# Zain-Jiang/Dict-TTS

Measured on AMD Instinct MI355X. Metric: mel-frames/sec, end-to-end text->mel->wav (audio-samples/sec = 256x; RTF reported alongside), higher is better.
Workload: dtype f16 (vocoder ResBlocks fp16 MFMA, serial convolutions bf16 hi/lo split; acoustic model fp32-grade: fp32 MFMA / bf16 three-piece operands x 6 products)

## Files before the change

### dict_tts_amd/csrc/rblock.hip

```cpp
#include "rblock.h"
#include "rb_common.h"
#include "rb_tiles.h"

#include <algorithm>
#include <type_traits>
#include <cstdlib>

namespace dtts {

#ifdef RB_STAMP
__device__ unsigned long long rb_stamps[2][12][16];
extern "C" __attribute__((visibility("default"))) int dtts_debug_rb_stamps(unsigned long long* host, int reset) {
    hipError_t e = hipMemcpyFromSymbol(host, HIP_SYMBOL(rb_stamps), sizeof(rb_stamps));
    if (e == hipSuccess && reset) {
        static unsigned long long z[2][12][16];
        e = hipMemcpyToSymbol(HIP_SYMBOL(rb_stamps), z, sizeof z);
    }
    return (int)e;
}
#define RB_T(k) do { const unsigned long long _n = __builtin_amdgcn_s_memrealtime(); tq[k] += _n - t_last; t_last = _n; } while (0)
#else
#define RB_T(k)
#endif

template <int C, int MT, int NT, int WT, int WC, int EL, int PS, bool GUARD, class SH = MfmaShape<32>>
__global__ __launch_bounds__(64 * WT * WC, (64 * WT * WC <= 256) ? 2 : 1) void rblock_kernel(const RBlockParams p) {
    static_assert(WC * NT * 32 == C, "channel tiling must cover C");
    typedef typename SH::acc_t acc_t;
    extern __shared__ __attribute__((aligned(16))) char smem[];
    constexpr int THREADS = 64 * WT * WC;
    constexpr int W = 32 * MT * WT;
    constexpr int PITCH = C * 2 + 16;
    constexpr int NKG = C / SH::CI;
    constexpr int EP = C * 4 + 16;
    constexpr int F4 = C / 4, SROWS = WT * 32;
    constexpr size_t ACT_BYTES = (size_t)(W + 2 * RB_GUARD) * PITCH;
    char* act = smem;
    char* stage = smem + ACT_BYTES;

    int tid = threadIdx.x, lane = tid & 63, wave = tid >> 6;
    int wt = wave % WT, wc = wave / WT;
    const int H = rblock_halo(p);
    const int TT = W - 2 * H;
    constexpr int PK = 7, PH = (PK - 1) / 2;
    const int TTo = p.wav ? TT - 2 * PH : TT;

    const RbTiles tiles{(int*)(smem + p.pre_off), p.B};
    auto zero_guard_bands = [&](int t) {
        for (int idx = t; idx < 2 * RB_GUARD * (PITCH / 16); idx += THREADS) {
            const int r = idx / (PITCH / 16), c = idx % (PITCH / 16);
            const int row = r < RB_GUARD ? r : W + r;
            *(uint4*)(act + row * PITCH + c * 16) = make_uint4(0, 0, 0, 0);
        }
    };
    zero_guard_bands(tid);
    int total = 0, j = blockIdx.x;
    if constexpr (PS) {
        tiles.build(p.lens, p.T, TTo, tid, THREADS);
        total = tiles.total();
        if (j >= total) return;
    }
    const int G = gridDim.x;

    typedef __attribute__((ext_vector_type(4))) unsigned int u32x4;
    constexpr int RPP = THREADS / F4;
    constexpr int PER = SROWS / RPP;
    static_assert(THREADS % F4 == 0 && SROWS % RPP == 0, "row-coalesced staging");
    int c4 = tid % F4, r0 = tid / F4;
    auto tile_row = [&](int m, int u) { const int sr = r0 + RPP * u; return ((sr >> 5) * MT + m) * 32 + (sr & 31); };

    auto load_x = [&](acc_t (&d)[NT], int m, int bb, int base, int ln) {
        const auto rs = __builtin_amdgcn_make_buffer_rsrc((void*)(p.x + (long long)bb * p.T * C), 0, ln * C * 4, 0x00020000);
        const int o0 = ((base + wt * MT * 32 + SH::row(lane, 0)) * C + wc * NT * 32 + SH::chan(lane, 0)) * 4;
#pragma unroll
        for (int n = 0; n < NT; ++n)
#pragma unroll
            for (int q = 0; q < 4; ++q) {
                const u32x4 v = __builtin_amdgcn_raw_buffer_load_b128(rs, o0 + (m * 32 * C + n * 32 + SH::row(0, q) * C + SH::chan(0, q)) * 4, 0, RB_X_AUX);
                SH::set_quad(d[n], q, __builtin_bit_cast(f32x4, v));
            }
    };

    int b = 0, len, t0;
    if constexpr (PS) {
        tiles.locate(j, b);
        len = tiles.len_of(b);
        t0 = tiles.first_row(j, b, TTo) - (p.wav ? PH : 0);
    } else {
        b = blockIdx.y;
        len = __builtin_amdgcn_readfirstlane(p.lens ? p.lens[b] : p.T);
        t0 = blockIdx.x * TTo - (p.wav ? PH : 0);
        if (t0 + (p.wav ? PH : 0) >= len) return;
    }
    acc_t xr[MT][NT];
    if constexpr (PS) {
#pragma unroll
        for (int m = 0; m < MT; ++m) load_x(xr[m], m, b, t0 - H, len);
    } else {
        const auto rs_x = __builtin_amdgcn_make_buffer_rsrc((void*)(p.x + (long long)b * p.T * C), 0, len * C * 4, 0x00020000);
        const int g0 = ((t0 - H + r0) * C + c4 * 4) * 4;
        u32x4 ld[MT][PER] = {};
#pragma unroll
        for (int m = 0; m < MT; ++m)
#pragma unroll
            for (int u = 0; u < PER; ++u) ld[m][u] = __builtin_amdgcn_raw_buffer_load_b128(rs_x, g0 + (tile_row(m, u) - r0) * (C * 4), 0, RB_X_AUX);
#pragma unroll
        for (int m = 0; m < MT; ++m) {
            if (m) __syncthreads();
#pragma unroll
            for (int u = 0; u < PER; ++u) *(u32x4*)(stage + (r0 + RPP * u) * EP + c4 * 16) = ld[m][u];
            __syncthreads();
#pragma unroll
            for (int n = 0; n < NT; ++n)
#pragma unroll
                for (int q = 0; q < 4; ++q)
                    SH::set_quad(xr[m][n], q, *(const f32x4*)(stage + (wt * 32 + SH::row(lane, q)) * EP + ((wc * NT + n) * 32 + SH::chan(lane, q)) * 4));
        }
    }

    const int kg_stride = (C / 32) * SH::WF * 64;
    int r = 0;

#ifdef RB_STAMP
    unsigned long long tq[16] = {0, 0, 0, 0, 0, 0, 0, 0, 0, 0, 0, 0, 0, 0, 0, 0};
    unsigned long long t_last = __builtin_amdgcn_s_memrealtime();
#endif
#pragma unroll 1
    for (;;) {
    if constexpr (PS) {
        tid = threadIdx.x;
        asm volatile("" : "+v"(tid));
        lane = tid & 63, wave = __builtin_amdgcn_readfirstlane(tid >> 6);
        wt = wave % WT, wc = wave / WT;
        c4 = tid % F4, r0 = tid / F4;
    }
    const int xlane = (RB_GUARD + wt * MT * 32 + SH::row(lane, 0)) * PITCH + SH::chan(lane, 0) * 4;
    const size_t wlane = (size_t)(wc * NT) * SH::WF * 64 + lane;
    if constexpr (PS) r = __builtin_amdgcn_readfirstlane(r);
    else r = 0;
    const RBlockParams::Set& R = p.rb[PS ? r : 0];
    const int Kr = R.K;
    constexpr bool REAL_STEPS = (C == 32);
    static_assert(!REAL_STEPS || SH::FRAG == 32, "rb2_contract is written for 32x32x16");
    static_assert(REAL_STEPS || NKG >= 4 || (NKG == 2 && SH::FRAG == 16), "whole groups of four k-steps, or rb_contract's half group");
    const int S = (REAL_STEPS ? Kr : R.Kp) * NKG;
    const bool last_rb = !PS || r + 1 == p.nrb;
    const int mode = (!PS || p.nrb == 1 || r == 0) ? p.mode : (last_rb ? p.last_mode : 1);
    const bool wav_now = p.wav && last_rb;
    t0 = __builtin_amdgcn_readfirstlane(t0);
    const int base_t = t0 - H;
    const long long brow = (long long)b * p.T;
    unsigned claim = 0;
    if (PS && p.tile_ctr && tid == 0 && last_rb) claim = atomicAdd(p.tile_ctr, 1u);
    int jn = j + G;
    bool has_next = PS && jn < total;
    int bn = b, lenn = len, t0n = 0;
    auto plan_next = [&]() {
        if (!last_rb) {
            has_next = true;
            jn = j;
            bn = b;
            lenn = len;
            t0n = t0;
            return;
        }
        has_next = PS && jn < total;
        bn = b;
        if (has_next) {
            tiles.locate(jn, bn);
            lenn = tiles.len_of(bn);
            t0n = tiles.first_row(jn, bn, TTo) - (p.wav ? PH : 0);
        }
    };
    if (!(PS && p.tile_ctr) || !last_rb) plan_next();
    const auto rs_s = p.s_private ? __builtin_amdgcn_make_buffer_rsrc((void*)p.S, 0, p.s_private, 0x00020000)
                                  : __builtin_amdgcn_make_buffer_rsrc((void*)(p.S + brow * C), 0, len * C * 4, 0x00020000);

    constexpr int NBQ = 4 / SH::QB;
    auto load_bias = [&](f32x4 (&bb)[NT][NBQ], const float* bias) {
#pragma unroll
        for (int n = 0; n < NT; ++n)
#pragma unroll
            for (int q = 0; q < NBQ; ++q) bb[n][q] = *(const f32x4*)(bias + (wc * NT + n) * 32 + SH::chan(lane, q * SH::QB));
    };
    const bool all_inb = base_t >= 0 && base_t + W <= len;
    int n_ovf = 0;
    auto write_act_impl = [&](char* dst, const acc_t (&v)[MT][NT], auto masked_tag) {
        constexpr bool MASKED = decltype(masked_tag)::value;
        int ln = lane;
        if constexpr (SH::FRAG == 16) asm volatile("" : "+v"(ln));
#pragma unroll
        for (int m = 0; m < MT; ++m) {
            int row[SH::QB];
            bool inb[SH::QB], counted[SH::QB];
#pragma unroll
            for (int rh = 0; rh < SH::QB; ++rh) {
                row[rh] = (wt * MT + m) * 32 + SH::row(ln, rh);
                const int t = base_t + row[rh];
                inb[rh] = !MASKED || (t >= 0 && t < len);
                counted[rh] = inb[rh] && row[rh] >= H && row[rh] < H + TT;
            }
#pragma unroll
            for (int n = 0; n < NT; ++n)
#pragma unroll
                for (int q = 0; q < 4; ++q) {
                    constexpr int QBM = SH::QB - 1;
                    const int co = (wc * NT + n) * 32 + SH::chan(ln, q);
                    const f32x4 v4 = SH::quad(v[m][n], q);
                    uint2 pk = act4<EL>(v4, 0.1f);
                    if constexpr (GUARD) n_ovf += counted[q & QBM] ? ovf4(v4, 0.1f) : 0;
                    if constexpr (MASKED) {
                        if (!inb[q & QBM]) pk = make_uint2(0, 0);
                    }
                    *(uint2*)(dst + (RB_GUARD + row[q & QBM]) * PITCH + co * 2) = pk;
                }
        }
    };
    auto write_act = [&](char* dst, const acc_t (&v)[MT][NT]) {
        if (all_inb) write_act_impl(dst, v, std::false_type{});
        else write_act_impl(dst, v, std::true_type{});
    };

    uint4 ring[SH::RD][NT * SH::WF];
    f32x4 bb[NT][NBQ];
    RB_T(10);
    rb_preload(ring, R.w1[0] + wlane, kg_stride);
    load_bias(bb, R.b1[0]);
    write_act(act, xr);
    RB_T(0);
    __syncthreads();
    RB_T(1);

    acc_t acc[MT][NT];
#pragma unroll 1
    for (int it = 0; it < 3; ++it) {
        acc_t cinit[NT];
#pragma unroll
        for (int n = 0; n < NT; ++n)
#pragma unroll
            for (int q = 0; q < 4; ++q) SH::set_quad(cinit[n], q, bb[n][q / SH::QB]);
        load_bias(bb, R.b2[it]);
        const int d = R.dil[it];
        if constexpr (REAL_STEPS) {
            if (S) rb2_contract<EL, MT, NT, NKG, PITCH, 4, true>(acc, ring, act, xlane - ((Kr - 1) / 2) * d * PITCH, R.w1[it] + wlane, S, d * PITCH, cinit);
            else rb_contract<EL, MT, NT, NKG, PITCH, true, 1>(acc, ring, act, 0, R.w1[it] + wlane, 0, 0, &cinit);
        } else
            rb_contract<EL, MT, NT, NKG, PITCH, true, 1, SH>(acc, ring, act, xlane - ((Kr - 1) / 2) * d * PITCH, R.w1[it] + wlane, S, d * PITCH, &cinit);
        rb_preload(ring, R.w2[it] + wlane, kg_stride);
        RB_T(2);
        __syncthreads();
        RB_T(3);
        write_act(act, acc);
        RB_T(4);
        __syncthreads();
        RB_T(5);
#pragma unroll
        for (int m = 0; m < MT; ++m)
#pragma unroll
            for (int n = 0; n < NT; ++n)
#pragma unroll
                for (int q = 0; q < 4; ++q) SH::add_quad(xr[m][n], q, bb[n][q / SH::QB]);
        if (it < 2) load_bias(bb, R.b1[it + 1]);
        if constexpr (REAL_STEPS) {
            if (S) rb2_contract<EL, MT, NT, NKG, PITCH, 4, false>(xr, ring, act, xlane - ((Kr - 1) / 2) * PITCH, R.w2[it] + wlane, S, PITCH, cinit);
        } else
            rb_contract<EL, MT, NT, NKG, PITCH, false, 1, SH>(xr, ring, act, xlane - ((Kr - 1) / 2) * PITCH, R.w2[it] + wlane, S, PITCH);
        if (it < 2) rb_preload(ring, R.w1[it + 1] + wlane, kg_stride);
        if (PS && p.tile_ctr && last_rb && it == 2 && tid == 0) tiles.publish_claim(G, claim);
        RB_T(6);
        __syncthreads();
        RB_T(7);
        if (it < 2) {
            write_act(act, xr);
            RB_T(0);
            __syncthreads();
            RB_T(1);
        }
    }

    if (PS && p.tile_ctr && last_rb) {
        jn = tiles.claimed();
        plan_next();
    }
    {
    const auto rs_a = __builtin_amdgcn_make_buffer_rsrc((void*)(p.Sa ? p.Sa + brow * C : (unsigned short*)(p.S + brow * C)), 0,
                                                        len * C * 2, 0x00020000);
    constexpr int CW = NT * 32, F4W = CW / 4, RPI = 64 / F4W, NRD = 32 / RPI;
    const int er = lane / F4W, ec = lane % F4W;
    const int goffw = (p.s_private ? (j * TT - H) * C : base_t * C) * 4 + (wc * CW + ec * 4) * 4;
    static_assert(F4W == 8 && RPI == 8 && NRD == 4, "the conflict-free row order below is for 8 lanes per row, 8 rows per access");
    const int erow_slab_base = C == 32 ? er : (er >> 2) + ((er & 1) ? 16 : 0) + ((er & 2) ? 8 : 0);
    auto srow = [&](int u) { return (C == 32 ? 8 : 2) * u + erow_slab_base; };
    auto erow = [&](int m, int u) { return (wt * MT + m) * 32 + srow(u); };
    auto eoff = [&](int m, int u) {
        const int row = erow(m, u);
        return (row >= H && row < H + TT) ? goffw + row * (C * 4) : (int)0x80000000;
    };
    u32x4 sold[MT][NRD];
#pragma unroll
    for (int m = 0; m < MT; ++m)
#pragma unroll
        for (int u = 0; u < NRD; ++u) {
            sold[m][u] = u32x4{0u, 0u, 0u, 0u};
            if (mode >= 1) sold[m][u] = p.nrb > 1 ? __builtin_amdgcn_raw_buffer_load_b128(rs_s, eoff(m, u), 0, 0)
                                                  : __builtin_amdgcn_raw_buffer_load_b128(rs_s, eoff(m, u), 0, VP_LD_AUX);
        }
    RB_T(12);
    constexpr int OP = C * 4;
    char* otile = smem;
    char* estage = wav_now ? smem + ((size_t)TT * OP > ACT_BYTES ? (size_t)TT * OP : ACT_BYTES) : stage;
    char* stg = estage + (wt * 32) * EP + (wc * CW) * 4;
#pragma unroll
    for (int m = 0; m < MT; ++m) {
#pragma unroll
        for (int n = 0; n < NT; ++n)
#pragma unroll
            for (int q = 0; q < 4; ++q) *(f32x4*)(stg + SH::row(lane, q) * EP + (n * 32 + SH::chan(lane, q)) * 4) = SH::quad(xr[m][n], q);
        if (has_next) load_x(xr[m], m, bn, t0n - H, lenn);
        __builtin_amdgcn_fence(__ATOMIC_RELEASE, "wavefront");
        __builtin_amdgcn_wave_barrier();
        __builtin_amdgcn_fence(__ATOMIC_ACQUIRE, "wavefront");
        RB_T(13);
#pragma unroll
        for (int u = 0; u < NRD; ++u) {
            const int off = eoff(m, u);
            f32x4 o = *(const f32x4*)(stg + srow(u) * EP + ec * 16);
            o += __builtin_bit_cast(f32x4, sold[m][u]);
            if (wav_now) {
                const int row = erow(m, u);
                if (row >= H && row < H + TT) {
                    const int t = base_t + row;
#pragma unroll
                    for (int e = 0; e < 4; ++e) o[e] = (t >= 0 && t < len) ? lrelu(o[e] / p.div, p.slope) : 0.f;
                    *(f32x4*)(otile + (size_t)(row - H) * OP + (wc * CW + ec * 4) * 4) = o;
                }
                continue;
            }
            rb_stage_row(o, rs_s, rs_a, off, mode, p.div, p.slope, p.drop_S != 0, p.Sa != nullptr, p.nrb > 1 && !last_rb);
        }
        __builtin_amdgcn_fence(__ATOMIC_RELEASE, "wavefront");
        __builtin_amdgcn_wave_barrier();
        __builtin_amdgcn_fence(__ATOMIC_ACQUIRE, "wavefront");
        RB_T(14);
    }
    if constexpr (C == 32) if (wav_now) {
        __syncthreads();
        rb_conv_post_tanh<C, THREADS, 3>(otile, p.post_w, p.post_b, p.wav + brow, t0, TTo, len, p.bad, tid);
    }
    }
    RB_T(8);
#ifdef RB_STAMP
    tq[11] += 1;
#endif
    if constexpr (GUARD) {
        if (n_ovf) atomicAdd(p.ovf, (unsigned long long)n_ovf);
    }
    if (!has_next) break;
    r = last_rb ? 0 : r + 1;
    if (wav_now) {
        __syncthreads();
        zero_guard_bands(threadIdx.x);
    }
    j = jn;
    b = bn;
    len = lenn;
    t0 = t0n;
    }
#ifdef RB_STAMP
    {
        const int w = threadIdx.x >> 6;
        if ((threadIdx.x & 63) == 0 && (w == 0 || w == WT * WC - 1)) {
            const int slot = (C == 32 ? 0 : C == 64 ? 1 : C == 128 ? 2 : 3) * 3 + (p.K == 3 ? 0 : p.K == 7 ? 1 : 2);
            for (int k = 0; k < 16; ++k) atomicAdd(&rb_stamps[w == 0 ? 0 : 1][slot][k], tq[k]);
        }
    }
#endif
}

template <int C, int MT, int WT>
static size_t rb_lds_bytes(int TT, bool wav) {
    constexpr int W = 32 * MT * WT, PITCH = C * 2 + 16, EP = C * 4 + 16;
    constexpr size_t ACT = (size_t)(W + 2 * RB_GUARD) * PITCH;
    if (wav)
        return std::max((size_t)TT * C * 4, ACT) + (size_t)WT * 32 * EP;
    return ACT + (size_t)WT * 32 * EP;
}

template <int C, int MT, int NT, int WT, int WC, int EL, int PS, bool GUARD = false>
static hipError_t rb_launch_cfg(const RBlockParams& p, hipStream_t stream) {
    typedef MfmaShape<rblock_mfma_shape(C)> SH;
    constexpr int W = 32 * MT * WT;
    for (int j = 0; j < p.nrb; ++j)
        if (!(p.rb[j].K & 1) || p.rb[j].Kp != rblock_padded_taps(C, p.rb[j].K)) return hipErrorInvalidValue;
    const int H = rblock_halo(p), TT = W - 2 * H;
    if (TT < 32) return hipErrorInvalidValue;
    if ((long long)p.T * C * 4 >= (1LL << 31)) return hipErrorInvalidValue;
    if (p.wav && (C != 32 || (p.nrb == 1 && p.mode != 2) || !p.post_w || !p.post_b)) return hipErrorInvalidValue;
    size_t lds = rb_lds_bytes<C, MT, WT>(TT, p.wav != nullptr);
    const int TTo = p.wav ? TT - 6 : TT;
    RBlockParams q = p;
    q.pre_off = (int)lds;
    if (PS) lds += rb_table_bytes(p.B);
    if (lds > 160 * 1024) return hipErrorOutOfMemory;
    constexpr bool HAS_GUARD = !(C == 64 && MT == 5);
    if constexpr (EL == EL_F16 && !GUARD && HAS_GUARD) {
        if (p.ovf) return rb_launch_cfg<C, MT, NT, WT, WC, EL, PS, true>(p, stream);
    }
    if (EL == EL_F16 && !HAS_GUARD && p.ovf) return hipErrorInvalidValue;
    constexpr auto kern = rblock_kernel<C, MT, NT, WT, WC, EL, PS, GUARD, SH>;
    if (const hipError_t e = rb_allow_full_lds<kern>(); e != hipSuccess) return e;
    constexpr int THREADS = 64 * WT * WC;
    if (!PS) {
        hipLaunchKernelGGL(kern, dim3((p.T + TTo - 1) / TTo, p.B), dim3(THREADS), lds, stream, q);
        return hipGetLastError();
    }
    const int cus = rb_device_cus();
    if (cus <= 0) return hipErrorInvalidDevice;
    const int grid = rb_resident_grid(cus, lds, THREADS, THREADS <= 256 ? 2 : 1, (long long)p.B * ((p.T + TTo - 1) / TTo));
    if (grid <= 0) return hipSuccess;
    hipLaunchKernelGGL(kern, dim3(grid), dim3(THREADS), lds, stream, q);
    return hipGetLastError();
}

bool rblock_supported(int C, int K) {
    if (!(K & 1) || K < 3 || K > 11) return false;
    return C == 32 || C == 64 || ((C == 128 || C == 256) && K == 3);
}

int rblock_stage_tile_rows(int C, int halo) {
    return (C == 32 ? 1024 : 512) - 2 * halo;
}

bool rblock_stage_launch_fits(int C, int halo, int B, bool wav) {
    const int TT = rblock_stage_tile_rows(C, halo);
    if (C != 32 && C != 64) return false;
    const size_t lds = (C == 32 ? rb_lds_bytes<32, 4, 8>(TT, wav) : rb_lds_bytes<64, 4, 4>(TT, wav)) + rb_table_bytes(B);
    return TT >= 32 && lds <= 160 * 1024;
}

long long rblock_private_rows(int C, int halo, int B, int T) {
    if (C != 32) return 0;
    const int TT = rblock_stage_tile_rows(C, halo), TTo = TT - 6;
    if (TTo < 32) return 0;
    return (long long)B * ((T + TTo - 1) / TTo) * TT;
}

int rblock_padded_taps(int C, int K) {
    const int sh = rblock_mfma_shape(C);
    const int nkg = C / (sh == 16 ? 32 : 16);
    if (sh == 16 && nkg == 2) return K;
    int kp = K;
    while ((kp * nkg) % 4) ++kp;
    return kp;
}

template <int EL>
static hipError_t rb_launch_el(const RBlockParams& p, int C, hipStream_t stream) {
    const int cus = rb_device_cus();
    if (cus <= 0) return hipErrorInvalidDevice;
    auto few = [&](int W) {
        const int tt = W - 2 * rblock_halo(p) - (p.wav ? 6 : 0);
        return tt >= 32 && 2 * (long long)p.B * ((p.T + tt - 1) / tt) <= cus;
    };
    if (p.nrb < 1 || p.nrb > 3) return hipErrorInvalidValue;
    if (p.nrb > 1) {
        if (C == 32) return rb_launch_cfg<32, 4, 1, 8, 1, EL, 1>(p, stream);
        if (C == 64) return rb_launch_cfg<64, 4, 1, 4, 2, EL, 1>(p, stream);
        return hipErrorInvalidValue;
    }
    if (C == 32 && p.K >= 7 && !few(1024)) RB_TRY((rb_launch_cfg<32, 4, 1, 8, 1, EL, 1>(p, stream)));
    if (C == 64 && few(512)) return rb_launch_cfg<64, 4, 1, 2, 2, EL, 1>(p, stream);
    if (C == 128 && few(256)) return rb_launch_cfg<128, 4, 1, 1, 4, EL, 1>(p, stream);
    if (C == 256 && few(128)) return rb_launch_cfg<256, 2, 1, 1, 8, EL, 1>(p, stream);
    if (C == 32) return rb_launch_cfg<32, 4, 1, 4, 1, EL, 0>(p, stream);
    if (C == 64 && p.K >= 7 && !p.small_tile && !(EL == EL_F16 && p.ovf)) RB_TRY((rb_launch_cfg<64, 5, 1, 4, 2, EL, 1>(p, stream)));
    if (C == 64) RB_TRY((rb_launch_cfg<64, 4, 1, 4, 2, EL, 1>(p, stream)));
    if (C == 64) return rb_launch_cfg<64, 4, 1, 2, 2, EL, 1>(p, stream);
    if (C == 128) RB_TRY((rb_launch_cfg<128, 4, 1, 2, 4, EL, 1>(p, stream)));
    if (C == 128) return rb_launch_cfg<128, 4, 1, 1, 4, EL, 1>(p, stream);
    if (C == 256) RB_TRY((rb_launch_cfg<256, 4, 1, 1, 8, EL, 1>(p, stream)));
    if (C == 256) return rb_launch_cfg<256, 2, 1, 1, 8, EL, 1>(p, stream);
    return hipErrorInvalidValue;
}

hipError_t rblock_launch(const RBlockParams& p, int C, int frag, hipStream_t stream) {
    if (C != 32 && C != 64 && C != 128 && C != 256) return hipErrorInvalidValue;
    if (frag != rblock_mfma_shape(C)) return hipErrorInvalidValue;
    return p.el == EL_F16 ? rb_launch_el<EL_F16>(p, C, stream) : rb_launch_el<EL_BF16>(p, C, stream);
}

}
```

### dict_tts_amd/csrc/vocoder.hip

```cpp
#include "ctx.h"

using namespace dtts;

namespace {

bool vocoder_fp16_analysis(dtts_ctx* h, Need& need) {
    const dtts_config& c = h->cfg;
    const std::string v = "vocoder.";
    const int nk = c.n_resblock_kernels;
    std::vector<double> pt_wc[2], pt_m2[2];
    for (int pass = 0; pass < 2; ++pass) {
        const double M = pass, bs = pass == 0 ? 1.0 : 0.0;
        auto conv = [&](const std::string& base, const std::vector<double>& uin, const std::vector<double>& min, std::vector<double>& uout,
                        std::vector<double>& mout) -> bool {
            const HostTensor* w = folded_weight(h, need, base);
            const std::vector<float> b = bias_of(need, base);
            if (!w || b.empty() || w->shape.size() != 3) return false;
            const int co_n = (int)w->shape[0], ci_n = (int)w->shape[1], k_n = (int)w->shape[2];
            if ((int)uin.size() < ci_n) return false;
            uout.assign(co_n, 0.0);
            mout.assign(co_n, 0.0);
            for (int co = 0; co < co_n; ++co) {
                double su = bs * std::fabs((double)b[co]), sm = bs * (double)b[co] * b[co];
                for (int ci = 0; ci < ci_n; ++ci) {
// ... 3 lines not shown
                        a1 += std::fabs((double)pw[k]);
                        a2 += (double)pw[k] * pw[k];
                    }
                    su += a1 * uin[ci];
                    sm += a2 * min[ci];
                }
                uout[co] = su;
                mout[co] = sm;
            }
            return true;
        };
        std::vector<double> u(c.audio_num_mel_bins, M), m(c.audio_num_mel_bins, M * M), u2, m2;
        if (!conv(v + "conv_pre", u, m, u2, m2)) return false;
        u.swap(u2);
        m.swap(m2);
        for (int i = 0; i < c.n_upsamples; ++i) {
            const int r = c.upsample_rates[i], k_n = c.upsample_kernel_sizes[i], pad = (k_n - r) / 2;
            const HostTensor* w = folded_weight(h, need, v + "ups." + std::to_string(i));
            const std::vector<float> b = bias_of(need, v + "ups." + std::to_string(i));
            if (!w || b.empty() || w->shape.size() != 3 || (int)w->shape[2] != k_n) return false;
            const int ci_n = (int)w->shape[0], co_n = (int)w->shape[1];
            std::vector<double> ux(co_n, 0.0), mx(co_n, 0.0);
            for (int co = 0; co < co_n; ++co)
                for (int ph = 0; ph < r; ++ph) {
                    double su = bs * std::fabs((double)b[co]), sm = bs * (double)b[co] * b[co];
                    for (int ci = 0; ci < ci_n; ++ci) {
                        const float* pw = &w->f[((size_t)ci * co_n + co) * k_n];
                        double a1 = 0, a2 = 0;
                        for (int k = (ph + pad) % r; k < k_n; k += r) {
                            a1 += std::fabs((double)pw[k]);
                            a2 += (double)pw[k] * pw[k];
                        }
                        su += a1 * u[ci];
                        sm += a2 * 0.505 * m[ci];
                    }
                    ux[co] = std::max(ux[co], su);
                    mx[co] = std::max(mx[co], sm);
                }
            std::vector<double> us(co_n, 0.0), ms(co_n, 0.0);
            for (int j = 0; j < nk; ++j) {
                std::vector<double> x = ux, xm = mx, xt, xtm, y, ym, xa(co_n), xam(co_n);
                const std::string rb = v + "resblocks." + std::to_string(i * nk + j);
                for (int mth = 0; mth < (h->resblock2 ? 2 : 3); ++mth) {
                    for (int q = 0; q < co_n; ++q) {
                        pt_wc[pass].push_back(x[q]);
                        pt_m2[pass].push_back(xm[q]);
                        xa[q] = x[q];
                        xam[q] = 0.505 * xm[q];
                    }
                    if (h->resblock2) {
                        if (!conv(rb + ".convs." + std::to_string(mth), xa, xam, y, ym)) return false;
                    } else {
                        if (!conv(rb + ".convs1." + std::to_string(mth), xa, xam, xt, xtm)) return false;
                        for (int q = 0; q < co_n; ++q) {
                            pt_wc[pass].push_back(xt[q]);
                            pt_m2[pass].push_back(xtm[q]);
                            xtm[q] *= 0.505;
                        }
                        if (!conv(rb + ".convs2." + std::to_string(mth), xt, xtm, y, ym)) return false;
                    }
                    for (int q = 0; q < co_n; ++q) {
                        x[q] += y[q];
                        xm[q] += ym[q];
                    }
                }
                for (int q = 0; q < co_n; ++q) {
                    us[q] += x[q] / nk;
                    ms[q] += xm[q] / nk;
                }
            }
            u.swap(us);
            m.swap(ms);
        }
    }
    if (pt_wc[0].size() != pt_wc[1].size()) return false;
    double a_wc = 0, b_wc = 0, a_m2 = 0, b_m2 = 0;
    for (size_t q = 0; q < pt_wc[0].size(); ++q) {
        a_wc = std::max(a_wc, pt_wc[0][q]);
        b_wc = std::max(b_wc, pt_wc[1][q]);
        a_m2 = std::max(a_m2, pt_m2[0][q]);
        b_m2 = std::max(b_m2, pt_m2[1][q]);
    }
    h->wc_const = a_wc;
    h->wc_lin = b_wc;
    h->est_const = std::sqrt(a_m2);
    h->est_lin = std::sqrt(b_m2);
    return true;
}

bool pack_rb_fused(dtts_ctx* h, Need& need, PackedConv& L, int eng, const std::string& base, int ch, int k, int dil, int frag) {
    const HostTensor* w = folded_weight(h, need, base);
    std::vector<float> bias = bias_of(need, base);
    if (!w || bias.empty()) return false;
    const float* pw = w->f.data();
    const int slack = ch >= 64 ? 1 : 2;
    const bool ok = pack_conv(h, L, eng, ch, ch, frag == RBN_FRAG ? rbn_padded_taps(ch, k) : rblock_padded_taps(ch, k) + slack,
                              [=](int co, int ci, int tap) { return tap < k ? pw[((size_t)co * ch + ci) * k + tap] : 0.f; }, bias, dil, 1, 0, 0, -1, frag);
    L.K = k;
    return ok;
}

bool vpair_pack_fits(const PackedConv& L, int ch, int k) {
    return L.C_in == ch && L.C_out == ch && L.C_in_pad == ch && L.C_out_pad == ch && L.K == k && L.frag == vpair_mfma_shape(ch);
}
bool vpair_runs(const dtts_config& c, bool resblock2, int eng_rb, int ch, int k, int d0, int d1, int d2) {
    const bool fuse = c.vocoder_precision == DTTS_VOC_F16 || !c.vocoder_unfused;
    return fuse && !resblock2 && eng_rb != ENG_BF16X3 && !rblock_supported(ch, k) && vpair_supported(ch, k, d0) && vpair_supported(ch, k, d1) &&
           vpair_supported(ch, k, d2);
}

}

namespace dtts {

int build_vocoder(dtts_ctx* h) {
    Need need{h, ""};
    const dtts_config& c = h->cfg;
    if (c.vocoder_precision != DTTS_VOC_BF16 && c.vocoder_precision != DTTS_VOC_BF16X3 && c.vocoder_precision != DTTS_VOC_F16)
        return fail(h, DTTS_E_INVAL, "vocoder_precision %d is not one of DTTS_VOC_BF16 / _BF16X3 / _F16", c.vocoder_precision);
    if (c.vocoder_precision == DTTS_VOC_F16 && c.audio_num_mel_bins % 4)
        return fail(h, DTTS_E_INVAL, "DTTS_VOC_F16 needs audio_num_mel_bins %% 4 == 0 (got %d); use DTTS_VOC_BF16X3", c.audio_num_mel_bins);
    if (!h->ovf_dev) {
        if (!(h->ovf_dev = (unsigned long long*)dev_alloc(h, sizeof(unsigned long long))) || hipMemset(h->ovf_dev, 0, sizeof(unsigned long long)) != hipSuccess)
            return fail(h, DTTS_E_NOMEM, "range-guard counter");
    }
    if (!h->bad_dev) {
        if (!(h->bad_dev = (unsigned*)dev_alloc(h, sizeof(unsigned))) || hipMemset(h->bad_dev, 0, sizeof(unsigned)) != hipSuccess)
            return fail(h, DTTS_E_NOMEM, "overflow-detector counter");
        void* hp = nullptr;
        if (hipHostMalloc(&hp, 64, hipHostMallocDefault) != hipSuccess) return fail(h, DTTS_E_NOMEM, "overflow-detector host word");
        h->bad_host = (volatile unsigned*)hp;
        *h->bad_host = 0;
    }
    const int eng = c.vocoder_precision == DTTS_VOC_BF16 ? ENG_BF16 : ENG_BF16X3;
    const int eng_rb = c.vocoder_precision == DTTS_VOC_F16 ? ENG_F16 : eng;
    const std::string v = "vocoder.";
    bool ok = pack_plain(h, need, h->conv_pre, eng, v + "conv_pre", 1, 1, 3);
    h->ups.resize(c.n_upsamples);
    h->hop = 1;
    for (int i = 0; ok && i < c.n_upsamples; ++i) {
        const int u = c.upsample_rates[i], k = c.upsample_kernel_sizes[i];
        const bool h2 = c.vocoder_precision == DTTS_VOC_F16 && i == 1 && DTTS_TUNE(h, 8192) && (u * (c.upsample_initial_channel >> (i + 1))) % 256 == 0 &&
                        (c.upsample_initial_channel >> i) % 128 == 0;
        ok = ok && pack_transposed(h, need, h->ups[i], h2 ? ENG_F16 : eng, v + "ups." + std::to_string(i), u, (k - u) / 2);
        h->hop *= u;
    }
    const int nk = c.n_resblock_kernels;
    h->rb1.assign((size_t)c.n_upsamples * nk, {});
    h->rb2.assign((size_t)c.n_upsamples * nk, {});
    const bool rb2x = h->resblock2;
    for (int i = 0; ok && i < c.n_upsamples * nk; ++i) {
        const int j = i % nk, k = c.resblock_kernel_sizes[j], n = rb2x ? 2 : 3;
        const int ch = c.upsample_initial_channel >> (i / nk + 1);
        const std::string r = v + "resblocks." + std::to_string(i);
        const int* dl = c.resblock_dilation_sizes[j];
        const bool vp = vpair_runs(c, rb2x, eng_rb, ch, k, dl[0], dl[1], dl[2]);
        const int frag = vp ? vpair_mfma_shape(ch) : 32;
        h->rb1[i].resize(n);
        if (!rb2x) h->rb2[i].resize(3);
        for (int mth = 0; ok && mth < n; ++mth) {
            const int d = c.resblock_dilation_sizes[j][mth];
            ok = ok && pack_plain(h, need, h->rb1[i][mth], eng_rb, r + (rb2x ? ".convs." : ".convs1.") + std::to_string(mth), d, 1, (k * d - d) / 2, true, 0, frag);
            if (!rb2x) ok = ok && pack_plain(h, need, h->rb2[i][mth], eng_rb, r + ".convs2." + std::to_string(mth), 1, 1, (k - 1) / 2, true, 0, frag);
            if (ok && vp && !vpair_pack_fits(h->rb1[i][mth], ch, k))
                return fail(h, DTTS_E_INVAL, "%s%d: weight shape [%d, %d, %d] is not the configured [%d, %d, %d]", (r + ".convs1.").c_str(), mth, h->rb1[i][mth].C_out,
                            h->rb1[i][mth].C_in, h->rb1[i][mth].K, ch, ch, k);
            if (ok && vp && !vpair_pack_fits(h->rb2[i][mth], ch, k))
                return fail(h, DTTS_E_INVAL, "%s%d: weight shape [%d, %d, %d] is not the configured [%d, %d, %d]", (r + ".convs2.").c_str(), mth, h->rb2[i][mth].C_out,
                            h->rb2[i][mth].C_in, h->rb2[i][mth].K, ch, ch, k);
        }
    }
    h->rbf1.assign((size_t)c.n_upsamples * nk, {});
    h->rbf2.assign((size_t)c.n_upsamples * nk, {});
    for (int i = 0; ok && rb2x && eng_rb != ENG_BF16X3 && i < c.n_upsamples * nk; ++i) {
        const int j = i % nk, k = c.resblock_kernel_sizes[j];
        const int ch = c.upsample_initial_channel >> (i / nk + 1);
        const int d0 = c.resblock_dilation_sizes[j][0], d1 = c.resblock_dilation_sizes[j][1];
        if (!rb2x_supported(ch, k, d0, d1) || h->rb1[i][0].C_in_pad != ch || nk < 2) {
            if (eng_rb == ENG_F16)
                return fail(h, DTTS_E_INVAL, "DTTS_VOC_F16 needs ResBlock2 widths 32/64/128/256, odd kernels 3..11 and a dilation pair whose halo fits the tile "
                            "(resblock %d: %d channels, k=%d, dilations (%d, %d)); use DTTS_VOC_BF16X3", i, ch, k, d0, d1);
            continue;
        }
        h->rbf1[i].resize(2);
        for (int mth = 0; ok && mth < 2; ++mth)
            ok = pack_rb_fused(h, need, h->rbf1[i][mth], eng_rb, v + "resblocks." + std::to_string(i) + ".convs." + std::to_string(mth), ch, k,
                               c.resblock_dilation_sizes[j][mth], 32);
    }
    for (int i = 0; ok && !rb2x && eng_rb != ENG_BF16X3 && i < c.n_upsamples * nk; ++i) {
        const int j = i % nk, k = c.resblock_kernel_sizes[j];
        const int ch = c.upsample_initial_channel >> (i / nk + 1);
        const int* dl = c.resblock_dilation_sizes[j];
        const bool narrow = nk >= 2 && rbn_supported(ch, k, dl[0], dl[1], dl[2]) && h->rb1[i][0].C_in == ch && h->rb1[i][0].C_out == ch;
        if (!rblock_supported(ch, k) && !narrow) {
            if (eng_rb == ENG_F16 && !vpair_runs(c, rb2x, eng_rb, ch, k, dl[0], dl[1], dl[2]))
                return fail(h, DTTS_E_INVAL, "DTTS_VOC_F16 needs ResBlock widths 8/16/32/64/128/256 and odd kernels 3..11 (resblock %d: %d channels, k=%d); use DTTS_VOC_BF16X3", i, ch, k);
            continue;
        }
        h->rbf1[i].resize(3);
        h->rbf2[i].resize(3);
        const std::string r = v + "resblocks." + std::to_string(i);
        const int ffrag = narrow ? RBN_FRAG : rblock_mfma_shape(ch);
        for (int mth = 0; ok && mth < 3; ++mth) {
            ok = pack_rb_fused(h, need, h->rbf1[i][mth], eng_rb, r + ".convs1." + std::to_string(mth), ch, k, c.resblock_dilation_sizes[j][mth], ffrag);
            ok = ok && pack_rb_fused(h, need, h->rbf2[i][mth], eng_rb, r + ".convs2." + std::to_string(mth), ch, k, 1, ffrag);
        }
    }
    ok = ok && pack_plain(h, need, h->conv_post, eng, v + "conv_post", 1, 1, 3);
    {
        const int last_ch = c.upsample_initial_channel >> c.n_upsamples;
        const HostTensor* w = ok ? folded_weight(h, need, v + "conv_post") : nullptr;
        const std::vector<float> b = ok ? bias_of(need, v + "conv_post") : std::vector<float>();
        bool fusable = ok && eng_rb != ENG_BF16X3 && (last_ch == 32 || (!rb2x && (last_ch == 16 || last_ch == 8))) && w && w->shape.size() == 3 && w->shape[0] == 1 &&
                       w->shape[1] == last_ch && w->shape[2] == 7 && b.size() == 1 && nk >= 2;
        for (int j = 0; fusable && j < nk; ++j) fusable = !h->rbf1[(size_t)(c.n_upsamples - 1) * nk + j].empty();
        if (fusable) {
            std::vector<float> wt((size_t)7 * last_ch);
            for (int ci = 0; ci < last_ch; ++ci)
                for (int k = 0; k < 7; ++k) wt[(size_t)k * last_ch + ci] = w->f[(size_t)ci * 7 + k];
            h->post_w = upload(h, wt);
            h->post_b = upload(h, b);
            ok = h->post_w && h->post_b;
        }
    }
    if (!ok) {
        if (!need.missing.empty()) return fail(h, DTTS_E_NOENT, "missing weight tensor '%s'", need.missing.c_str());
        if (h->err.empty()) return fail(h, DTTS_E_NOMEM, "packing / uploading vocoder weights failed");
        return DTTS_E_INVAL;
    }
    if (c.vocoder_precision == DTTS_VOC_F16 && !vocoder_fp16_analysis(h, need)) return fail(h, DTTS_E_NOENT, "fp16 analysis: missing weight tensor '%s'", need.missing.c_str());
    h->vocoder_ready = true;
    return DTTS_OK;
}

}

namespace {

struct StageGeom {
    long long rows[9];
    int ch[9];
    size_t max_elems;
};
StageGeom stage_geom(const dtts_config& c, int B, int T) {
    StageGeom g;
    g.rows[0] = T;
    g.ch[0] = c.upsample_initial_channel;
    g.max_elems = (size_t)B * T * g.ch[0];
    for (int i = 0; i < c.n_upsamples; ++i) {
        g.rows[i + 1] = g.rows[i] * c.upsample_rates[i];
        g.ch[i + 1] = g.ch[i] / 2;
        g.max_elems = std::max<size_t>(g.max_elems, (size_t)B * (size_t)g.rows[i + 1] * (size_t)g.ch[i + 1]);
    }
    return g;
}

struct StageMult { int m[9]; };

__global__ void zero_wav_tails_kernel(float* wav, const int32_t* lens, int T, int hop) {
    const int b = blockIdx.y;
    const long long n = (long long)T * hop;
    int l = lens[b];
    l = l < 0 ? 0 : (l > T ? T : l);
    const long long first = (long long)l * hop;
    const long long i = first + ((long long)blockIdx.x * blockDim.x + threadIdx.x) * 4;
    if (i + 3 < n) *(float4*)(wav + (long long)b * n + i) = make_float4(0.f, 0.f, 0.f, 0.f);
    else for (long long k = i; k < n; ++k) wav[(long long)b * n + k] = 0.f;
}

}

extern "C" __global__ void scale_lens_kernel(const int32_t* lens, int32_t* out, int B, int T, int n_stage, StageMult mult) {
    const int i = blockIdx.x * blockDim.x + threadIdx.x;
    if (i >= B * n_stage) return;
    const int sidx = i / B, b = i % B;
    int l = lens ? lens[b] : T;
    l = l < 0 ? 0 : (l > T ? T : l);
    out[i] = l * mult.m[sidx];
}

namespace {

void scale_lens(const dtts_config& c, const int32_t* lens, int* lensS, int B, int T, hipStream_t s) {
    const int nup = c.n_upsamples;
    StageMult mult;
    mult.m[0] = 1;
    for (int i = 0; i < nup; ++i) mult.m[i + 1] = mult.m[i] * c.upsample_rates[i];
    hipLaunchKernelGGL(scale_lens_kernel, dim3((B * (nup + 1) + 255) / 256), dim3(256), 0, s, lens, lensS, B, T, nup + 1, mult);
}


enum RbPath { RB_WHOLE, RB_VPAIR, RB_CONVS };
RbPath rb_path(const dtts_ctx* h, bool fuse, int ch, size_t rb) {
    if (fuse && !h->rbf1[rb].empty()) return RB_WHOLE;
    if (h->resblock2) return RB_CONVS;
    const auto& c1 = h->rb1[rb];
    return fuse && vpair_runs(h->cfg, false, c1[0].engine, ch, c1[0].K, c1[0].dil, c1[1].dil, c1[2].dil) ? RB_VPAIR : RB_CONVS;
}

struct FusePlan {
    int fuse_n[8];
    size_t s_elems;
};
FusePlan fuse_plan(const dtts_ctx* h, const StageGeom& g, int B, bool fuse) {
    const dtts_config& c = h->cfg;
    const int nup = c.n_upsamples, nk = c.n_resblock_kernels;
    FusePlan pl = {{1, 1, 1, 1, 1, 1, 1, 1}, g.max_elems};
    for (int i = 0; i < nup; ++i) {
        const long long rows = g.rows[i + 1];
        const int ch = g.ch[i + 1];
        if (h->resblock2) continue;
        if (fuse && DTTS_TUNE(h, 4096) && !DTTS_TUNE(h, 512) && nk == 3 && ch == 32 && !h->rbf1[(size_t)i * nk].empty() && !h->rbf1[(size_t)i * nk + 1].empty()) {
            int halo2 = 0;
            for (int j = 0; j < 2; ++j) halo2 = std::max(halo2, rblock_halo_of(h->rbf1[(size_t)i * nk + j][0].K, c.resblock_dilation_sizes[j]));
            const int TT2 = rblock_stage_tile_rows(ch, halo2);
            if (TT2 >= 64 && rblock_stage_launch_fits(ch, halo2, B, false) && (long long)B * ((rows + TT2 - 1) / TT2) >= 2LL * h->n_cu) pl.fuse_n[i] = 2;
            continue;
        }
        bool all = fuse && DTTS_TUNE(h, 512) && nk >= 2 && nk <= 3 && (ch == 32 || ch == 64);
        int halo = 0;
        for (int j = 0; j < nk && all; ++j) {
            all = !h->rbf1[(size_t)i * nk + j].empty();
            if (all) halo = std::max(halo, rblock_halo_of(h->rbf1[(size_t)i * nk + j][0].K, c.resblock_dilation_sizes[j]));
        }
        if (!all) continue;
        const bool with_post = i == nup - 1 && h->post_w;
        const int TT = rblock_stage_tile_rows(ch, halo);
        if (TT < 64 || !rblock_stage_launch_fits(ch, halo, B, with_post) || (long long)B * ((rows + TT - 1) / TT) < 2LL * h->n_cu) continue;
        if (with_post) {
            const long long prow = rblock_private_rows(ch, halo, B, (int)rows);
            if (prow <= 0 || (size_t)prow * ch * sizeof(float) >= (size_t)INT_MAX) continue;
            pl.s_elems = std::max(pl.s_elems, (size_t)prow * ch);
        }
        pl.fuse_n[i] = nk;
    }
    return pl;
}

typedef unsigned short bf;
constexpr int TV = DTTS_TIMER_VOC_CONV;
constexpr int N_CTR = 64;

struct VocRun {
    dtts_ctx* h;
    hipStream_t s;
    int B, nk;
    bool exact;
    int el;
    float* wav;
    float *Xf, *Rf, *Sf, *Rg;
    bf *Xa, *Ra, *Ta, *Sa;
    unsigned* ctrs;
    int n_ctr;
    size_t s_cap_bytes;
    bool post_done;
    int i, ch, Tcur;
    const int* lout;
    bool last_stage;

    template <class P>
    void whole_rb_params(P& rp, int j, int j_last) {
        memset(&rp, 0, sizeof rp);
        rp.x = Xf;
        rp.S = Sf;
        rp.lens = lout;
        rp.B = B;
        rp.T = Tcur;
        rp.mode = j == 0 ? 0 : (j == nk - 1 ? 2 : 1);
        rp.div = (float)nk;
        rp.slope = last_stage ? 0.01f : 0.1f;
        rp.Sa = exact ? nullptr : Sa;
        rp.drop_S = exact ? 0 : 1;
        if (last_stage && j_last == nk - 1 && h->post_w) {
            rp.wav = wav;
            rp.post_w = h->post_w;
            rp.post_b = h->post_b;
            rp.Sa = nullptr;
            post_done = true;
        }
        rp.el = el;
        rp.tile_ctr = n_ctr < N_CTR ? ctrs + n_ctr++ : nullptr;
        rp.ovf = (exact && h->guard_on) ? h->ovf_dev : nullptr;
        rp.bad = h->bad_dev;
    }

    int rblock(int j, int fuse_n) {
        if (nk == 1) return fail(h, DTTS_E_INVAL, "fused ResBlock path needs >= 2 resblock kernels");
        if (j > 0 && j < fuse_n) return DTTS_OK;
        const int j_last = j == 0 ? fuse_n - 1 : j;
        RBlockParams rp;
        whole_rb_params(rp, j, j_last);
        rp.nrb = j_last - j + 1;
        rp.last_mode = j_last == nk - 1 ? 2 : 1;
        int frag = 0;
        for (int jj = j; jj <= j_last; ++jj) {
            RBlockParams::Set& st = rp.rb[jj - j];
            const auto& g1 = h->rbf1[(size_t)i * nk + jj];
            const auto& g2 = h->rbf2[(size_t)i * nk + jj];
            st.K = g1[0].K;
            st.Kp = rblock_padded_taps(ch, g1[0].K);
            if (jj == j) frag = g1[0].frag;
            for (int mth = 0; mth < 3; ++mth)
                if (g1[mth].frag != frag || g2[mth].frag != frag) frag = 0;
            for (int mth = 0; mth < 3; ++mth) {
                st.w1[mth] = (const uint4*)g1[mth].w_hi;
                st.w2[mth] = (const uint4*)g2[mth].w_hi;
                st.b1[mth] = g1[mth].bias;
                st.b2[mth] = g2[mth].bias;
                st.dil[mth] = g1[mth].dil;
            }
            rp.K = std::max(rp.K, st.K);
        }
        if (rp.wav && fuse_n == nk) rp.s_private = (int)std::min<size_t>(s_cap_bytes, (size_t)INT_MAX);
        rp.small_tile = DTTS_TUNE(h, 16384) ? 1 : 0;
        if (h->debug_misorder) frag = frag == 16 ? 32 : 16;
        Timed tm(h, TV, s);
        LAUNCH(rblock_launch(rp, ch, frag, s));
        return DTTS_OK;
    }

    int rbn(int j) {
        const auto& g1 = h->rbf1[(size_t)i * nk + j];
        const auto& g2 = h->rbf2[(size_t)i * nk + j];
        RBnParams rp;
        whole_rb_params(rp, j, j);
        rp.K = g1[0].K;
        rp.Kp = rbn_padded_taps(ch, g1[0].K);
        int frag = g1[0].frag;
        for (int mth = 0; mth < 3; ++mth) {
            if (g1[mth].frag != frag || g2[mth].frag != frag) frag = 0;
            rp.w1[mth] = (const uint4*)g1[mth].w_hi;
            rp.w2[mth] = (const uint4*)g2[mth].w_hi;
            rp.b1[mth] = g1[mth].bias;
            rp.b2[mth] = g2[mth].bias;
            rp.dil[mth] = g1[mth].dil;
        }
        if (h->debug_misorder) frag = 16;
        Timed tm(h, TV, s);
        LAUNCH(rbn_launch(rp, ch, frag, s));
        return DTTS_OK;
    }

    int rb2x(int j) {
        const auto& fv = h->rbf1[(size_t)i * nk + j];
        RB2xParams rp;
        whole_rb_params(rp, j, j);
        rp.K = fv[0].K;
        rp.Kp = rblock_padded_taps(ch, fv[0].K);
        for (int m = 0; m < 2; ++m) {
            rp.w[m] = (const uint4*)fv[m].w_hi;
            rp.b[m] = fv[m].bias;
            rp.dil[m] = fv[m].dil;
        }
        Timed tm(h, TV, s);
        LAUNCH(rb2x_launch(rp, ch, s));
        return DTTS_OK;
    }

    int vpair(int j) {
        const auto& c1 = h->rb1[(size_t)i * nk + j];
        const auto& c2 = h->rb2[(size_t)i * nk + j];
        for (int mth = 0; mth < 3; ++mth)
            if (!vpair_pack_fits(c1[mth], ch, c1[0].K) || !vpair_pack_fits(c2[mth], ch, c1[0].K))
                return fail(h, DTTS_E_STATE, "resblock %d is not packed for vpair<%d>", i * nk + j, ch);
        const float* xin = Xf;
        for (int mth = 0; mth < 3; ++mth) {
            VPairParams vp;
            memset(&vp, 0, sizeof vp);
            vp.x = xin;
            vp.w1 = (const uint4*)c1[mth].w_hi;
            vp.w2 = (const uint4*)c2[mth].w_hi;
            vp.b1 = c1[mth].bias;
            vp.b2 = c2[mth].bias;
            vp.lens = lout;
            vp.B = B;
            vp.T = Tcur;
            vp.K = c1[mth].K;
            vp.dil = c1[mth].dil;
            vp.div = (float)nk;
            vp.slope = last_stage ? 0.01f : 0.1f;
            vp.el = el;
            vp.tile_ctr = n_ctr < N_CTR ? ctrs + n_ctr++ : nullptr;
            vp.ovf = (exact && h->guard_on) ? h->ovf_dev : nullptr;
            const bool s16 = exact && !DTTS_TUNE(h, 32768);
            vp.x16 = (s16 && mth > 0) ? 1 : 0;
            if (mth < 2) {
                vp.y = mth == 0 ? Rf : Rg;
                vp.mode = 1;
                vp.y16 = s16 ? 1 : 0;
            } else {
                vp.y = Sf;
                vp.mode = j == 0 ? 1 : (j == nk - 1 ? 3 : 2);
                vp.ya = exact ? nullptr : Sa;
                vp.drop_y = exact ? 0 : 1;
            }
            xin = vp.y;
            Timed tm(h, TV, s);
            LAUNCH(vpair_launch(vp, ch, s));
        }
        return DTTS_OK;
    }

    int convs(int j) {
        if (exact) return fail(h, DTTS_E_STATE, "DTTS_VOC_F16: resblock %d has no fused kernel", i * nk + j);
        const auto& c1 = h->rb1[(size_t)i * nk + j];
        if (c1[0].frag != 32) return fail(h, DTTS_E_STATE, "resblock %d is packed for vpair, not for the per-convolution kernels", i * nk + j);
        const int n = h->resblock2 ? 2 : 3;
        for (int mth = 0; mth < n; ++mth) {
            const bf* xa = mth == 0 ? Xa : Ra;
            if (!h->resblock2) {
                VConvParams p = vparams(c1[mth], xa, lout, B, Tcur);
                p.ldx = ch;
                p.ya = Ta;
                p.ldya = ch;
                p.slope = 0.1f;
                Timed tm(h, TV, s);
                LAUNCH(vconv_launch(p, s));
                xa = Ta;
            }
            VConvParams p = vparams(h->resblock2 ? c1[mth] : h->rb2[(size_t)i * nk + j][mth], xa, lout, B, Tcur);
            p.ldx = ch;
            p.res = mth == 0 ? Xf : Rf;
            p.ldres = ch;
            if (mth < n - 1) {
                p.yf = Rf;
                p.ldyf = ch;
                p.ya = Ra;
                p.ldya = ch;
                p.slope = 0.1f;
            } else {
                p.yf = Sf;
                p.ldyf = ch;
                if (j > 0) {
                    p.res2 = Sf;
                    p.ldres2 = ch;
                }
                if (j == nk - 1) {
                    p.div = (float)nk;
                    p.ya = Sa;
                    p.ldya = ch;
                    p.slope = last_stage ? 0.01f : 0.1f;
                }
            }
            Timed tm(h, TV, s);
            LAUNCH(vconv_launch(p, s));
        }
        return DTTS_OK;
    }
};

int hifigan_forward_fused(dtts_ctx* h, const float* mel, const int32_t* lens, int B, int T, float* wav, hipStream_t s) {
    const dtts_config& c = h->cfg;
    const bool exact = c.vocoder_precision == DTTS_VOC_F16;
    const int nup = c.n_upsamples, nk = c.n_resblock_kernels;
    const int melC = h->conv_pre.C_in_pad;
    const bool fuse = exact || !c.vocoder_unfused;
    const StageGeom g = stage_geom(c, B, T);
    const FusePlan plan = fuse_plan(h, g, B, fuse);
    const size_t max_elems = g.max_elems, s_elems = plan.s_elems;
    HIPCHK(h->a_voc.reserve((s_elems - max_elems) * sizeof(float) + max_elems * (4 * sizeof(float) + 4 * sizeof(bf)) + (size_t)B * T * melC * sizeof(bf) +
                            (size_t)(nup + 2) * B * sizeof(int) + (64 << 10), s));
    Arena& A = h->a_voc;
    VocRun r = {h, s, B, nk, exact, exact ? EL_F16 : EL_BF16, wav};
    r.s_cap_bytes = s_elems * sizeof(float);
    float* Xf = r.Xf = A.alloc<float>(max_elems);
    r.Rf = A.alloc<float>(max_elems);
    float* Sf = r.Sf = A.alloc<float>(s_elems);
    r.Rg = A.alloc<float>(max_elems);
    bf* Xa = r.Xa = A.alloc<bf>(max_elems);
    r.Ra = A.alloc<bf>(max_elems);
    r.Ta = A.alloc<bf>(max_elems);
    bf* Sa = r.Sa = A.alloc<bf>(max_elems);
    bf* melb = A.alloc<bf>((size_t)B * T * melC);
    int* lensS = A.alloc<int>((size_t)(nup + 1) * B);
    r.ctrs = A.alloc<unsigned>(N_CTR);
    if (!Xf || !r.Rf || !Sf || !r.Rg || !Xa || !r.Ra || !r.Ta || !Sa || !melb || !lensS || !r.ctrs) return fail(h, DTTS_E_NOMEM, "vocoder workspace");
    HIPCHK(hipMemsetAsync(r.ctrs, 0, N_CTR * sizeof(unsigned), s));
    scale_lens(c, lens, lensS, B, T, s);
    if (lens && (h->hop & 3) == 0 && ((uintptr_t)wav & 15) == 0) {
        const long long n = (long long)T * h->hop;
        hipLaunchKernelGGL(zero_wav_tails_kernel, dim3((unsigned)((n / 4 + 255) / 256), B), dim3(256), 0, s, wav, lens, T, h->hop);
        HIPCHK(hipGetLastError());
    } else if (lens) HIPCHK(hipMemsetAsync(wav, 0, (size_t)B * T * h->hop * sizeof(float), s));
    struct SpanGuard {
        dtts_ctx* h;
        Timed* t;
        ~SpanGuard() {
            h->voc_span = false;
            delete t;
        }
    } span{h, nullptr};
    if (h->timers[TV].enabled) {
        span.t = new Timed(h, TV, s);
        if (span.t->e1) h->timers[TV].launches -= 1;
        h->voc_span = true;
    }
    if (exact) {
        VConvParams p = vparams_x3(h->conv_pre, mel, c.audio_num_mel_bins, 1.f, lensS, B, T);
        p.yf = Sf;
        p.ldyf = g.ch[0];
        Timed tm(h, TV, s);
        LAUNCH(vconv_launch(p, s));
    } else {
        LAUNCH(f32_to_bf16_pad_launch(mel, melb, (long long)B * T, c.audio_num_mel_bins, melC, s));
        VConvParams p = vparams(h->conv_pre, melb, lensS, B, T);
        p.ya = Sa;
        p.ldya = g.ch[0];
        p.slope = 0.1f;
        Timed tm(h, TV, s);
        LAUNCH(vconv_launch(p, s));
    }
    for (int i = 0; i < nup; ++i) {
        const int u = c.upsample_rates[i], ch = g.ch[i + 1], Tin = (int)g.rows[i];
        const int* lin = lensS + (size_t)i * B;
        bool need_xa = false;
        for (int j = 0; j < nk; ++j) need_xa = need_xa || rb_path(h, fuse, ch, (size_t)i * nk + j) == RB_CONVS;
        {
            VConvParams p = exact ? vparams_x3(h->ups[i], Sf, 2 * ch, 0.1f, lin, B, Tin) : vparams(h->ups[i], Sa, lin, B, Tin);
            if (!exact) p.ldx = 2 * ch;
            p.small_tiles = exact;
            p.yf = Xf;
            p.ldyf = u * ch;
            p.ya = need_xa ? Xa : nullptr;
            p.ldya = u * ch;
            p.slope = 0.1f;
            Timed tm(h, TV, s);
            LAUNCH(vconv_launch(p, s));
        }
        r.i = i;
        r.ch = ch;
        r.Tcur = (int)g.rows[i + 1];
        r.lout = lensS + (size_t)(i + 1) * B;
        r.last_stage = i == nup - 1;
        for (int j = 0; j < nk; ++j) {
            const RbPath path = rb_path(h, fuse, ch, (size_t)i * nk + j);
            const bool narrow = path == RB_WHOLE && !h->resblock2 && h->rbf1[(size_t)i * nk + j][0].frag == RBN_FRAG;
            const int rc = path == RB_WHOLE ? (h->resblock2 ? r.rb2x(j) : (narrow ? r.rbn(j) : r.rblock(j, plan.fuse_n[i])))
                                            : (path == RB_VPAIR ? r.vpair(j) : r.convs(j));
            if (rc) return rc;
        }
    }
    if (!r.post_done) {
        const int Tcur = (int)g.rows[nup], ch = g.ch[nup];
        VConvParams p = exact ? vparams_x3(h->conv_post, Sf, ch, 0.01f, lensS + (size_t)nup * B, B, Tcur)
                              : vparams(h->conv_post, Sa, lensS + (size_t)nup * B, B, Tcur);
        if (!exact) p.ldx = ch;
        p.yf = wav;
        p.ldyf = 1;
        p.post_tanh = 1;
        p.bad = h->bad_dev;
        Timed tm(h, TV, s);
        LAUNCH(vconv_launch(p, s));
    }
    return DTTS_OK;
}

int hifigan_forward_x3(dtts_ctx* h, const float* mel, const int32_t* lens, int B, int T, float* wav, hipStream_t s) {
    const dtts_config& c = h->cfg;
    const int nup = c.n_upsamples, nk = c.n_resblock_kernels;
    const size_t max_elems = stage_geom(c, B, T).max_elems;
    HIPCHK(h->a_voc.reserve(4 * (max_elems * sizeof(float) + 256) + (size_t)(nup + 2) * B * sizeof(int) + 8192, s));
    float* bufX = h->a_voc.alloc<float>(max_elems);
    float* bufR = h->a_voc.alloc<float>(max_elems);
    float* bufT = h->a_voc.alloc<float>(max_elems);
    float* bufS = h->a_voc.alloc<float>(max_elems);
    int* lensS = h->a_voc.alloc<int>((size_t)(nup + 1) * B);
    if (!bufX || !bufR || !bufT || !bufS || !lensS) return fail(h, DTTS_E_NOMEM, "vocoder workspace");
    scale_lens(c, lens, lensS, B, T, s);
    int Tcur = T, ch = c.upsample_initial_channel;
    {
        ConvParams p = base_params(mel, c.audio_num_mel_bins, B, T, T, bufS, ch);
        p.in_lens = lensS;
        p.out_lens = lensS;
        Timed tm(h, TV, s);
        LAUNCH(conv1d_launch(h->conv_pre, p, s));
    }
    for (int i = 0; i < nup; ++i) {
        const int u = c.upsample_rates[i];
        const int* lin = lensS + (size_t)i * B;
        const int* lout = lensS + (size_t)(i + 1) * B;
        ch /= 2;
        {
            ConvParams p = base_params(bufS, 2 * ch, B, Tcur, Tcur, bufX, u * ch);
            p.in_lens = lin;
            p.out_lens = lin;
            p.pre_act = 1;
            p.pre_slope = 0.1f;
            Timed tm(h, TV, s);
            LAUNCH(conv1d_launch(h->ups[i], p, s));
        }
        Tcur *= u;
        auto conv = [&](const PackedConv& L, const float* xin, const float* res, float* y, bool last, int j) -> int {
            ConvParams p = base_params(xin, ch, B, Tcur, Tcur, y, ch);
            p.in_lens = lout;
            p.out_lens = lout;
            p.pre_act = 1;
            p.pre_slope = 0.1f;
            if (res) set_res(p, 0, res, ch);
            if (last && j > 0) {
                p.seg[0].res2 = bufS;
                p.seg[0].ld_res2 = ch;
            }
            if (last && j == nk - 1) p.out_div = (float)nk;
            Timed tm(h, TV, s);
            LAUNCH(conv1d_launch(L, p, s));
            return DTTS_OK;
        };
        for (int j = 0; j < nk; ++j) {
            const auto& c1 = h->rb1[(size_t)i * nk + j];
            const int n = h->resblock2 ? 2 : 3;
            for (int mth = 0; mth < n; ++mth) {
                const float* xin = mth == 0 ? bufX : bufR;
                const bool last = mth == n - 1;
                if (!h->resblock2)
                    if (int rc = conv(c1[mth], xin, nullptr, bufT, false, j)) return rc;
                const PackedConv& L = h->resblock2 ? c1[mth] : h->rb2[(size_t)i * nk + j][mth];
// ... 98 lines not shown
```

Measured before the change: 1.332 million.

## Split fused ResBlock stage launches across utterance ranges instead of one launch

The fused multi-ResBlock stage used to run as one launch over the whole batch while the other ResBlock slots did nothing. Now each ResBlock slot j below fuse_n launches the fused kernel over its own slice of utterances, with the x, S, lens and wav pointers offset to that slice. The private S strips used by the post-conv path are offset to match. The fit and occupancy checks are rescaled to the per-slice batch, so fusion can turn off for small batches. The overflow counting now excludes the post-conv halo rows when wav is written. This adds launches and changes how fused stages are chosen, and it assumes the slices stay non-empty and fit in the buffer.

```diff
diff --git a/dict_tts_amd/csrc/rblock.hip b/dict_tts_amd/csrc/rblock.hip
--- a/dict_tts_amd/csrc/rblock.hip
+++ b/dict_tts_amd/csrc/rblock.hip
@@ -198,7 +198,7 @@
                 row[rh] = (wt * MT + m) * 32 + SH::row(ln, rh);
                 const int t = base_t + row[rh];
                 inb[rh] = !MASKED || (t >= 0 && t < len);
-                counted[rh] = inb[rh] && row[rh] >= H && row[rh] < H + TT;
+                counted[rh] = inb[rh] && row[rh] >= H + (p.wav ? PH : 0) && row[rh] < H + TT - (p.wav ? PH : 0);
             }
 #pragma unroll
             for (int n = 0; n < NT; ++n)
diff --git a/dict_tts_amd/csrc/vocoder.hip b/dict_tts_amd/csrc/vocoder.hip
--- a/dict_tts_amd/csrc/vocoder.hip
+++ b/dict_tts_amd/csrc/vocoder.hip
@@ -329,6 +329,10 @@
     int fuse_n[8];
     size_t s_elems;
 };
+inline void fuse_range(int B, int n, int r, int& b0, int& b1) {
+    b0 = (int)((long long)B * r / n);
+    b1 = (int)((long long)B * (r + 1) / n);
+}
 FusePlan fuse_plan(const dtts_ctx* h, const StageGeom& g, int B, bool fuse) {
     const dtts_config& c = h->cfg;
     const int nup = c.n_upsamples, nk = c.n_resblock_kernels;
@@ -341,7 +345,8 @@
             int halo2 = 0;
             for (int j = 0; j < 2; ++j) halo2 = std::max(halo2, rblock_halo_of(h->rbf1[(size_t)i * nk + j][0].K, c.resblock_dilation_sizes[j]));
             const int TT2 = rblock_stage_tile_rows(ch, halo2);
-            if (TT2 >= 64 && rblock_stage_launch_fits(ch, halo2, B, false) && (long long)B * ((rows + TT2 - 1) / TT2) >= 2LL * h->n_cu) pl.fuse_n[i] = 2;
+            if (TT2 >= 64 && rblock_stage_launch_fits(ch, halo2, (B + 1) / 2, false) && (long long)(B / 2) * ((rows + TT2 - 1) / TT2) >= 2LL * h->n_cu)
+                pl.fuse_n[i] = 2;
             continue;
         }
         bool all = fuse && DTTS_TUNE(h, 512) && nk >= 2 && nk <= 3 && (ch == 32 || ch == 64);
@@ -353,7 +358,7 @@
         if (!all) continue;
         const bool with_post = i == nup - 1 && h->post_w;
         const int TT = rblock_stage_tile_rows(ch, halo);
-        if (TT < 64 || !rblock_stage_launch_fits(ch, halo, B, with_post) || (long long)B * ((rows + TT - 1) / TT) < 2LL * h->n_cu) continue;
+        if (TT < 64 || !rblock_stage_launch_fits(ch, halo, (B + nk - 1) / nk, with_post) || (long long)(B / nk) * ((rows + TT - 1) / TT) < 2LL * h->n_cu) continue;
         if (with_post) {
             const long long prow = rblock_private_rows(ch, halo, B, (int)rows);
             if (prow <= 0 || (size_t)prow * ch * sizeof(float) >= (size_t)INT_MAX) continue;
@@ -413,10 +418,26 @@
 
     int rblock(int j, int fuse_n) {
         if (nk == 1) return fail(h, DTTS_E_INVAL, "fused ResBlock path needs >= 2 resblock kernels");
-        if (j > 0 && j < fuse_n) return DTTS_OK;
-        const int j_last = j == 0 ? fuse_n - 1 : j;
+        const bool split = j < fuse_n && fuse_n > 1;
+        const int range = j;
+        int b0 = 0, b1 = B;
+        if (split) {
+            fuse_range(B, fuse_n, range, b0, b1);
+            j = 0;
+        }
+        const int j_last = split ? fuse_n - 1 : j;
         RBlockParams rp;
         whole_rb_params(rp, j, j_last);
+        if (split) {
+            if (b1 <= b0) return fail(h, DTTS_E_STATE, "fused stage: empty utterance range %d of %d (B = %d)", range, fuse_n, B);
+            const size_t off = (size_t)b0 * Tcur * ch;
+            rp.x = Xf + off;
+            rp.S = Sf + off;
+            if (rp.Sa) rp.Sa += off;
+            rp.lens = lout + b0;
+            rp.B = b1 - b0;
+            if (rp.wav) rp.wav = wav + (size_t)b0 * Tcur;
+        }
         rp.nrb = j_last - j + 1;
         rp.last_mode = j_last == nk - 1 ? 2 : 1;
         int frag = 0;
@@ -438,7 +459,14 @@
             }
             rp.K = std::max(rp.K, st.K);
         }
-        if (rp.wav && fuse_n == nk) rp.s_private = (int)std::min<size_t>(s_cap_bytes, (size_t)INT_MAX);
+        if (rp.wav && split && fuse_n == nk) {
+            const int halo = rblock_halo(rp);
+            const size_t first = (size_t)rblock_private_rows(ch, halo, b0, Tcur) * ch, count = (size_t)rblock_private_rows(ch, halo, b1 - b0, Tcur) * ch;
+            if (!count || (first + count) * sizeof(float) > s_cap_bytes || count * sizeof(float) >= (size_t)INT_MAX)
+                return fail(h, DTTS_E_STATE, "fused stage: the private strips of range %d do not fit the stage-sum buffer", range);
+            rp.S = Sf + first;
+            rp.s_private = (int)(count * sizeof(float));
+        }
         rp.small_tile = DTTS_TUNE(h, 16384) ? 1 : 0;
         if (h->debug_misorder) frag = frag == 16 ? 32 : 16;
         Timed tm(h, TV, s);
```

Result: no change. 1.331 million (median of 2 runs) (-0.1%).
